# if001/lit-llama-ja

Hardware: AMD Instinct MI355X
Metric: decode tokens/sec LLaMA-7B gptq.int4 bs=1, 1xMI355X per replica (higher is better)
Workload: dtype bf16; 1 GPU; LLaMA-7B --quantize gptq.int4 greedy decode, batch 1, prompt 16, max_seq_length 144; batch_per_gpu=1, prompt_len=16, max_seq_length=144, parallelism=replicas x1 (no collective on the data path)

## Files before the change

### __graft_entry__.py

```python
from __future__ import annotations

import sys
from pathlib import Path

REPO = Path(__file__).resolve().parent
PKG_ROOT = REPO / "lit-llama-ja_amd"
for _p in (str(REPO), str(PKG_ROOT)):
    if _p not in sys.path:
        sys.path.insert(0, _p)


def build() -> None:
    from lit_llama._build import build as _build

    so = _build(force=True, verbose=True)
    import lit_llama
    from lit_llama import _hip

    L = _hip.lib()
    print(f"built {so} ({so.stat().st_size} bytes); {len(_hip.SIGNATURES) + len(_hip.LORA_SIGNATURES) + len(_hip.NLL_SIGNATURES) + 1} entry points resolved")


def smoke() -> None:
    import numpy as np
    import torch

    import generate as G
    from lit_llama import LLaMA, LLaMAConfig
    from lit_llama.utils import EmptyInitOnDevice
    from oracle import llama_np as O
    from oracle.weights import Cfg, make_params

    assert torch.cuda.is_available(), "smoke() needs the GPU"
    g = dict(np.load(REPO / "tests" / "golden" / "int4_gptq.npz"))
    cfg = Cfg(block_size=128, n_layer=2, n_head=4, n_embd=256, vocab_size=2048)
    params = make_params(cfg, int(g["seed"]))
    packed = {k[3:]: v for k, v in g.items() if k.startswith("sd/")}
    with EmptyInitOnDevice(device=torch.device("cuda:0"), dtype=torch.bfloat16, quantization_mode="gptq.int4"):
        model = LLaMA(LLaMAConfig(block_size=128, vocab_size=2048, n_layer=2, n_head=4, n_embd=256))
    sd = {k: torch.from_numpy(v) for k, v in params.items() if not (k.endswith(".weight") and "wte" not in k)}
    sd.update({k: torch.from_numpy(np.ascontiguousarray(v)) for k, v in packed.items()})
    model.load_state_dict(sd)
    prompt = torch.from_numpy(g["prompt"]).cuda()
    ids = G.generate(model, prompt, 8, top_k=1).cpu().numpy()
    ref = g["bf16_ids"][: len(ids)]
    assert (ids == ref).all(), f"greedy ids {ids} != reference {ref}"
    lin = {k[:-len(".quant_weight")]: O.LinearSpec("colblock", qw=v, scales=packed[k[:-12] + "scales"],
                                                    zeros=packed[k[:-12] + "zeros"], bits=4)
           for k, v in packed.items() if k.endswith(".quant_weight")}
    orc = O.OracleLLaMA(cfg, params, linears=lin)
    want = orc.forward(g["prompt"][None].astype(np.int64))[0, -1]
    model.reset_cache()
    got = model(prompt[None].long())[0, -1].float().cpu().numpy()
# ... 8 lines not shown
```

### include/lit_llama_amd.h

```cpp
#ifndef LIT_LLAMA_AMD_H
#define LIT_LLAMA_AMD_H

#include <stddef.h>

#ifdef __cplusplus
extern "C" {
#endif

#define LLJ_EINVAL 1000

int llj_w4_repack(const void* qweight_ref, void* packed, int N, int K, void* stream);
int llj_w4_unpack(const void* packed, void* qweight_ref, int N, int K, void* stream);

int llj_w4_scale_zero(const void* scales, const void* zeros, int dtype, void* sz, int N, void* stream);

int llj_w8_repack(const void* qweight_ref, void* packed, int N, int K, void* stream);
int llj_w8_unpack(const void* packed, void* qweight_ref, int N, int K, void* stream);
int llj_w8_scale_zero(const void* scales, const void* zeros, int dtype, void* sz, int N, void* stream);

int llj_i8_repack(const void* cb, void* packed, int N, int K, void* stream);
int llj_i8_unpack(const void* packed, void* cb, int N, int K, void* stream);

int llj_set_tpw_max(int tiles);

// ... 151 lines not shown
int llj_g_sample(const float* logits, int ldl, int M, int V, float temperature, int top_k, const float* u,
                 unsigned long long seed, int* out_idx, int* tokens_out, int tok_stride, const int* pos, void* stream);

size_t llj_i8_rowstats_bytes(int K);
int llj_attention_i8(const void* q, const void* kcache, const void* vcache, void* y, const int* pos, int B, int T,
                     int n_head, int head_size, int S, int nsplit, void* part_ws, void* y_stats, void* clr,
                     int clr_words, float threshold, void* stream);
int llj_i8_swiglu_stats(const void* x, const void* CB1, const void* SCB1, const void* CB2, const void* SCB2, void* h,
                        int M, int H, int K, const void* i8ws, const void* x_stats, void* h_stats, void* clr,
                        int clr_words, float threshold, void* stream);
#define LLJ_WF_I8_ROWSTATS 0x10000
int llj_i8_norm_rowstats(const void* x, const void* norm_w, float eps, void* xn, int M, int K, float threshold, void* ws,
                         void* st, void* stream);
int llj_i8_linear_resid(const void* A, int lda, const void* CB, const void* SCB, void* x, int ldx, int M, int N, int K,
                        const void* stats, void* stream);

int llj_attention_adapter(const void* q, const void* kcache, const void* vcache, void* y, const int* pos, int B, int T,
                          int n_head, int head_size, int S, const void* ak, const void* av, const float* gate, int aT,
                          void* stream);
int llj_adapter_prefix_add(const void* q, const void* ak, const void* av, const float* gate, void* y, int M, int n_head,
                           int head_size, int aT, int dt, void* stream);

int llj_stream_read(const void* p, size_t bytes, float* out, int grid, void* stream);


#ifdef __cplusplus
}
#endif

#include "lit_llama_amd_lora.h"

#include "lit_llama_amd_nll.h"

#endif
```

### lit-llama-ja_amd/csrc/gemv.hip

```cpp
#include "gemv_impl.h"

namespace llj {

int g_tpw_max = LLJ_TPW_MAX;
int g_stream_a = 1;

template <int EP>
static int dispatch(int wf, int am, const GemvParams& p, hipStream_t s) {
  if (p.lora.t) {
    if (EP != EP_QKV || p.ad_s) return LLJ_EINVAL;
    switch (wf) {
      case WF_W4: return gemv_launch_lora_w4(am, p, s);
      case WF_BF16: return gemv_launch_lora_bf16(am, p, s);
      case WF_W8: return gemv_launch_lora_w8(am, p, s);
      case WF_W4G: return gemv_launch_lora_w4g(am, p, s);
    }
    return LLJ_EINVAL;
  }
  if (p.ad_s) {
    switch (wf) {
      case WF_W4: return gemv_launch_aff_w4(am, EP, p, s);
      case WF_BF16: return gemv_launch_aff_bf16(am, EP, p, s);
      case WF_W8: return gemv_launch_aff_w8(am, EP, p, s);
      case WF_W4G: return gemv_launch_aff_w4g(am, EP, p, s);
// ... 40 lines not shown
  const int old = g_tpw_max;
  g_tpw_max = tiles < 1 ? 1 : tiles;
  return old;
}

int llj_set_stream_a(int mode) {
  const int old = g_stream_a;
  g_stream_a = mode < 0 ? 0 : mode > 2 ? 2 : mode;
  return old;
}

int llj_linear(int wfmt, const void* A, int lda, const void* W, const void* sz, const void* bias, void* C,
               int ldc, int M, int N, int K, const void* i8ws, int i8_row0, const float* rowsum, void* stream) {
  GemvParams p{};
  p.rowsum = rowsum;
  p.A = (const bf16_t*)A; p.lda = lda; p.M = M; p.N = N; p.K = K;
  p.W = W; p.sz = (const float2*)sz; p.bias = (const bf16_t*)bias; p.C = (bf16_t*)C; p.ldc = ldc;
  p.i8ws = i8ws; p.m0 = i8_row0;
  return run<EP_STORE>(wfmt, p, stream);
}

int llj_norm_linear(int wfmt, const void* x, const void* norm_w, float eps, const void* W, const void* sz,
                    void* out, int ldo, int M, int N, int K, const void* i8ws, int i8_row0, const float* rowsum,
                    const float* nstat, int npart, void* stream) {
  GemvParams p{};
  p.rowsum = rowsum;
  p.nstat = nstat; p.npart = npart;
  p.A = (const bf16_t*)x; p.lda = K; p.norm_w = (const bf16_t*)norm_w; p.eps = eps; p.M = M; p.N = N; p.K = K;
  p.W = W; p.sz = (const float2*)sz; p.C = (bf16_t*)out; p.ldc = ldo;
  p.i8ws = i8ws; p.m0 = i8_row0;
  return run<EP_STORE>(wfmt, p, stream);
}

int llj_linear_resid(int wfmt, const void* A, int lda, const void* W, const void* sz, void* x, int ldx, int M,
                     int N, int K, const void* i8ws, int i8_row0, float* nstat_out, void* stream) {
  GemvParams p{};
  p.nstat_out = nstat_out;
  p.A = (const bf16_t*)A; p.lda = lda; p.M = M; p.N = N; p.K = K;
  p.W = W; p.sz = (const float2*)sz; p.C = (bf16_t*)x; p.ldc = ldx;
  p.i8ws = i8ws; p.m0 = i8_row0;
  return run<EP_RESID>(wfmt, p, stream);
}

int llj_norm_swiglu(int wfmt, const void* x, const void* norm_w, float eps, const void* W1, const void* sz1,
                    const void* W2, const void* sz2, void* h, int M, int H, int K, const void* i8ws, int i8_row0,
                    const float* rowsum, const float* nstat, int npart, void* stream) {
  GemvParams p{};
  p.rowsum = rowsum;
  p.nstat = nstat; p.npart = npart;
  p.A = (const bf16_t*)x; p.lda = K; p.norm_w = (const bf16_t*)norm_w; p.eps = eps; p.M = M; p.N = H; p.K = K;
  p.W = W1; p.W2 = W2; p.sz = (const float2*)sz1; p.sz2 = (const float2*)sz2; p.C = (bf16_t*)h; p.ldc = H;
  p.i8ws = i8ws; p.m0 = i8_row0;
  return run<EP_SWIGLU>(wfmt, p, stream);
}

int llj_norm_qkv_rope(int wfmt, const void* x, const void* norm_w, float eps, const void* W, const void* sz,
                      void* q_out, void* kcache, void* vcache, const float* rope, const int* pos, int B, int T,
                      int C, int n_head, int S, int row0, int rows, const void* i8ws, const float* rowsum,
                      const float* nstat, int npart, void* stream) {
  GemvParams p{};
  p.rowsum = rowsum ? rowsum + row0 : nullptr;
  p.nstat = nstat ? nstat + row0 : nullptr; p.npart = npart;
  if (row0 < 0 || rows < 1 || row0 + rows > B * T || n_head < 1 || C % n_head || S < 1) return LLJ_EINVAL;
  p.A = (const bf16_t*)x + (size_t)row0 * C; p.lda = C; p.norm_w = (const bf16_t*)norm_w; p.eps = eps;
  p.M = rows; p.m0 = row0; p.N = 3 * C; p.K = C;
  p.W = W; p.sz = (const float2*)sz; p.q_out = (bf16_t*)q_out; p.kcache = (bf16_t*)kcache;
// ... 160 lines not shown
```

### lit-llama-ja_amd/csrc/gemv_impl.h

```cpp
#pragma once
#include <algorithm>

#include "common.h"
#include "i8ws.h"
#include "attention.h"
#include "lit_llama_amd.h"

namespace llj {

enum : int { WF_W4 = 0, WF_BF16 = 1, WF_I8 = 2, WF_W8 = 3, WF_W4G = 4 };
enum : int { AM_GLOBAL = 0, AM_LDS = 1, AM_NORM = 2, AM_STREAM = 3, AM_SNORM = 4, AM_I8Q = 5, AM_I8S = 6, AM_MERGE = 7 };
constexpr int kMergeMax = 4;
constexpr int kSRow = 136;
constexpr int kSSlot = 8 * kSRow;
__host__ __device__ constexpr bool am_stream(int am) { return am == AM_STREAM || am == AM_SNORM; }
constexpr int kQRow = 144;
constexpr int kQSlotBytes = 8 * kQRow + 128 * 32;
constexpr int kQSlotBytesS = 8 * kQRow;
enum : int { EP_STORE = 0, EP_RESID = 1, EP_QKV = 2, EP_SWIGLU = 3 };


struct GemvParams {
  const bf16_t* A;
  int lda;
// ... 2 lines not shown
  int M, N, K;
  const void* W;
  const void* W2;
  const float2* sz;
  const float2* sz2;
  const bf16_t* bias;
  bf16_t* C;
  int ldc;
  bf16_t* q_out;
  bf16_t* kcache;
  bf16_t* vcache;
  const float* rope;
  const int* pos;
  int n_head, head_size, S, T;
  int m0;
  const void* i8ws;
  const float* rowsum;
  const float* nstat;
  int npart;
  float* nstat_out;
  int gch;
  const uint32_t* i8st;
  uint32_t* i8st_out;
  uint32_t* clr;
  int clr_words;
  float thr;
  const float* apart;
  int asplit;
  const bf16_t* ad_s;
  const bf16_t* ad_b;
  const bf16_t* ad_s2;
  const bf16_t* ad_b2;
  LoraArgs lora;
};
constexpr int kNstRows = 16;

__device__ __forceinline__ float rms_rstd(float sumsq_over_k, float eps) {
  return round_bf(rsqrtf(round_bf(round_bf(sumsq_over_k) + eps)));
}

__device__ __forceinline__ uint4 norm8(uint4 x, uint4 g, float r) {
  uint32_t xw[4] = {x.x, x.y, x.z, x.w}, gw[4] = {g.x, g.y, g.z, g.w}, o[4];
#pragma unroll
  for (int i = 0; i < 4; ++i) o[i] = cvt_pk(unpk(gw[i]) * unpk(cvt_pk(unpk(xw[i]) * r)));
  return make_uint4(o[0], o[1], o[2], o[3]);
}
__device__ __forceinline__ f32x2 sumsq8(const u32x4 x, f32x2 acc) {
#pragma unroll
  for (int i = 0; i < 4; ++i) {
    const f32x2 v = unpk(x[i]);
    acc += unpk(cvt_pk(v * v));
  }
  return acc;
}

template <int NW, bool NORM>
__device__ void stage_a(const GemvParams& p, bf16_t* As, int a_stride, float* red) {
  const int tid = threadIdx.x;
  constexpr int NT = NW * 64;
  const int K = p.K, M = p.M;
  const int nvec = K >> 3;
  float ss[8];
#pragma unroll
  for (int m = 0; m < 8; ++m) ss[m] = 0.f;
  const bool from_stat = NORM && p.nstat;
#pragma unroll
// ... 1236 lines not shown
        const int b = p.T == 1 ? mg : mg / p.T;
        float out = v;
        if (region < 2) out = (dd & 1) ? (v * cs.x + partner * cs.y) : (v * cs.x - partner * cs.y);
        const uint32_t ob = (uint32_t)f2bf(out);
        const uint32_t pr = lane_xor1(ob);
        if (!(dd & 1)) {
          bf16_t* dst;
          size_t ei;
          if (region == 0) {
            dst = p.q_out;
            ei = (size_t)mg * Cd + nc;
          } else {
            int slot = ps;
            if (slot >= p.S) slot %= p.S;
            dst = region == 1 ? p.kcache : p.vcache;
            ei = (((size_t)b * p.n_head + h) * p.S + slot) * p.head_size + dd;
          }
          epi_store(dst + ei, ob | (pr << 16));
        }
      }
    } else if (EP == EP_RESID) {
      const float xn = round_bf(bf2f(xr) + round_bf(y));
      const uint32_t xb = (uint32_t)f2bf(xn);
      const uint32_t pr = lane_xor1(xb);
      if (act && !(row & 1)) epi_store(p.C + (size_t)m * p.ldc + n, xb | (pr << 16));
      if (p.nstat_out) {
        const float sq = row16_sum(act ? round_bf(xn * xn) : 0.f);
        if (row == 0 && act) epi_store(p.nstat_out + (size_t)nt * kNstRows + m, __builtin_bit_cast(uint32_t, sq));
      }
    } else {
      const uint32_t ob = (uint32_t)f2bf(out_value<EP>(y, y2));
      const uint32_t pr = lane_xor1(ob);
      if (act && !(row & 1)) epi_store(p.C + (size_t)m * p.ldc + n, ob | (pr << 16));
      if constexpr (EP == EP_SWIGLU && I8) {
        if (p.i8st_out) {
          const float a16 = fabsf(f16r(bflo(ob)));
          big = act && a16 >= p.thr;
          const float mx = row16_max(act && !big ? a16 : 0.f);
          if (row == 0 && act) atomicMax(p.i8st_out + kI8StSca + 8 * (nt % kI8StSlots) + m, __float_as_uint(mx));
        }
      }
    }
    return big;
  };

  if constexpr ((LLJ_ABL & 4) != 0) {
    if (wave == 0 && acc[0][0] == 1234.5f && row < M) p.C[nj[0]] = f2bf(acc[0][1] + acc2[0][2]);
  } else if constexpr (FLAT) {
#pragma unroll
    for (int q = 0; q < FQ; ++q) {
      const int j = f_j[q], m = f_m[q];
      const int src = ((m >> 2) << 4) | row, r = m & 3;
      float ya = 0.f, yb = 0.f, ys = 0.f;
      int yi = 0, yi2 = 0;
#pragma unroll
      for (int w = 0; w < NW; ++w) {
        const float* o = red + (size_t)(w * 64 + src) * NV;
        if constexpr (I8) {
          const int* oi = reinterpret_cast<const int*>(o);
          yi = w == 0 ? oi[r] : yi + oi[r];
          yi2 = w == 0 ? oi[4 + r] : yi2 + oi[4 + r];
        } else {
          ya = w == 0 ? o[8 * j + r] : ya + o[8 * j + r];
          if (DUAL) yb = w == 0 ? o[8 * j + 4 + r] : yb + o[8 * j + 4 + r];
          if (SACC) ys = w == 0 ? o[8 * TPW + r] : ys + o[8 * TPW + r];
        }
// ... 303 lines not shown
```

### lit-llama-ja_amd/csrc/ops.hip

```cpp
#include <cstdlib>

#include "common.h"
#include "attention.h"
#include "lit_llama_amd.h"

namespace llj {

__global__ __launch_bounds__(256) void embedding_kernel(const int* __restrict__ idx, const uint4* __restrict__ wte,
                                                        uint4* __restrict__ out, int C8, int* pos_inc) {
  const int m = blockIdx.x;
  const size_t r = (size_t)idx[m];
  for (int v = threadIdx.x; v < C8; v += blockDim.x) out[(size_t)m * C8 + v] = wte[r * C8 + v];
  if (pos_inc && m == 0 && threadIdx.x == 0) *pos_inc += 1;
}

__global__ __launch_bounds__(256) void embedding_any_kernel(const int* __restrict__ idx, const bf16_t* __restrict__ wte,
                                                            bf16_t* __restrict__ out, int C, int* pos_inc) {
  const int m = blockIdx.x;
  const size_t r = (size_t)idx[m];
  for (int v = threadIdx.x; v < C; v += blockDim.x) out[(size_t)m * C + v] = wte[r * C + v];
  if (pos_inc && m == 0 && threadIdx.x == 0) *pos_inc += 1;
}


// ... 62 lines not shown

template <int HS, int U, int NTH, int SPECU>
__global__ __launch_bounds__(NTH) void attention_kernel(const bf16_t* __restrict__ q, const bf16_t* __restrict__ kc,
                                                        const bf16_t* __restrict__ vc, bf16_t* __restrict__ y,
                                                        const int* __restrict__ pos, int T, int S, int nh,
                                                        float scale_log2, uint32_t* st, float thr, uint32_t* clr,
                                                        int clr_words, int spec_ok) {
  __shared__ float lds[attention_lds_floats<HS, NTH>()];
  attention_body<HS, U, NTH, false, SPECU>(q, kc, vc, y, pos, T, S, nh, scale_log2, blockIdx.x, blockIdx.y, lds, 1, 0,
                                           nullptr, st, thr, clr, clr_words, spec_ok != 0);
}

template <int HS, int U, int NTH>
__global__ __launch_bounds__(NTH) void attention_part_kernel(const bf16_t* __restrict__ q, const bf16_t* __restrict__ kc,
                                                             const bf16_t* __restrict__ vc, const int* __restrict__ pos,
                                                             int T, int S, int nh, float scale_log2, int nsplit,
                                                             float* __restrict__ part) {
  __shared__ float lds[attention_lds_floats<HS, NTH>()];
  attention_body<HS, U, NTH, true>(q, kc, vc, nullptr, pos, T, S, nh, scale_log2, blockIdx.x, blockIdx.y, lds, nsplit,
                                   blockIdx.z, part);
}

template <int HS, int U, int NTH, int SPECU>
__global__ __launch_bounds__(NTH) void attention_ilv_kernel(const bf16_t* __restrict__ q, const bf16_t* __restrict__ kc,
                                                            const bf16_t* __restrict__ vc, const int* __restrict__ pos,
                                                            int T, int S, int nh, float scale_log2, int nsplit,
                                                            float* __restrict__ part, int spec_ok) {
  __shared__ float lds[attention_lds_floats<HS, NTH>()];
  attention_body<HS, U, NTH, true, SPECU, true>(q, kc, vc, nullptr, pos, T, S, nh, scale_log2, blockIdx.x, blockIdx.y,
                                                lds, nsplit, blockIdx.z, part, nullptr, 0.f, nullptr, 0,
                                                spec_ok != 0);
}

__global__ __launch_bounds__(1024) void argmax_kernel(const bf16_t* __restrict__ logits, int ldl, int V,
                                                      int* __restrict__ out_idx, int* __restrict__ tokens_out,
                                                      int tok_stride, const int* __restrict__ pos) {
  __shared__ float sv[16];
  __shared__ int si[16];
  const int m = blockIdx.x, tid = threadIdx.x;
  const bf16_t* lr = logits + (size_t)m * ldl;
  float best = -INFINITY;
  int bi = 0x7fffffff;
  auto take = [&](float x, int v) {
    if (x > best || (x == best && v < bi)) { best = x; bi = v; }
  };
  if ((V & 7) == 0 && (ldl & 7) == 0 && (reinterpret_cast<uintptr_t>(lr) & 15) == 0) {
    const uint4* l4 = reinterpret_cast<const uint4*>(lr);
    const int nv = V >> 3;
    for (int v0 = tid; v0 < nv; v0 += 4 * 1024) {
      uint4 r[4];
#pragma unroll
      for (int u = 0; u < 4; ++u) {
        const int v = v0 + 1024 * u;
        r[u] = l4[v < nv ? v : v0];
      }
#pragma unroll
      for (int u = 0; u < 4; ++u) {
        const int v = v0 + 1024 * u;
        if (v < nv) {
          const uint32_t w[4] = {r[u].x, r[u].y, r[u].z, r[u].w};
#pragma unroll
          for (int i = 0; i < 4; ++i) {
            take(bflo(w[i]), 8 * v + 2 * i);
            take(bfhi(w[i]), 8 * v + 2 * i + 1);
          }
        }
      }
    }
  } else {
    for (int v = tid; v < V; v += 1024) take(bf2f(lr[v]), v);
  }
#pragma unroll
  for (int o = 32; o > 0; o >>= 1) {
    const float ov = __shfl_xor(best, o, 64);
    const int oi = __shfl_xor(bi, o, 64);
    if (ov > best || (ov == best && oi < bi)) { best = ov; bi = oi; }
  }
  if ((tid & 63) == 0) { sv[tid >> 6] = best; si[tid >> 6] = bi; }
  __syncthreads();
  if (tid == 0) {
    for (int w = 1; w < 16; ++w)
      if (sv[w] > best || (sv[w] == best && si[w] < bi)) { best = sv[w]; bi = si[w]; }
    if (bi == 0x7fffffff) bi = 0;
    out_idx[m] = bi;
    if (tokens_out) tokens_out[(size_t)m * tok_stride + pos[0] + 1] = bi;
  }
}


__device__ __forceinline__ uint32_t bf_key(uint32_t b) { return (b & 0x8000u) ? (~b & 0xFFFFu) : (b | 0x8000u); }
__device__ __forceinline__ float key_bf(uint32_t k) {
  const uint32_t b = (k & 0x8000u) ? (k & 0x7FFFu) : (~k & 0xFFFFu);
  return bf2f((bf16_t)b);
}
__device__ __forceinline__ uint64_t splitmix64(uint64_t z) {
  z += 0x9E3779B97F4A7C15ull;
  z = (z ^ (z >> 30)) * 0xBF58476D1CE4E5B9ull;
  z = (z ^ (z >> 27)) * 0x94D049BB133111EBull;
  return z ^ (z >> 31);
}

constexpr int kSampNT = 1024;
__device__ __forceinline__ uint32_t block_suffix_excl(uint32_t v, uint32_t* wsum) {
  const int lane = threadIdx.x & 63, wv = threadIdx.x >> 6;
  uint32_t x = v;
#pragma unroll
  for (int o = 1; o < 64; o <<= 1) {
    const uint32_t y = (uint32_t)__shfl_down((int)x, o, 64);
    if (lane + o < 64) x += y;
  }
  if (lane == 0) wsum[wv] = x;
  __syncthreads();
  uint32_t above = 0;
  for (int w = wv + 1; w < kSampNT / 64; ++w) above += wsum[w];
  __syncthreads();
  return x - v + above;
}

template <typename T>
struct SampTraits;
template <>
// ... 308 lines not shown
                     int clr_words, float threshold, void* stream) {
  LLJ_REQUIRE(y_stats && B * T <= 8 && clr_words >= 0 && (!clr_words || clr));
  return attention_split_run(q, kcache, vcache, y, pos, B, T, n_head, head_size, S, nsplit, part_ws,
                             (uint32_t*)y_stats, threshold, (uint32_t*)clr, clr_words, stream);
}

int llj_sample(const void* logits, int ldl, int M, int V, float temperature, int top_k, const float* u,
               unsigned long long seed, int* out_idx, int* tokens_out, int tok_stride, const int* pos, void* stream) {
  LLJ_REQUIRE(M > 0 && V > 0 && temperature > 0.f && (!tokens_out || pos) && (u || pos));
  hipLaunchKernelGGL(sample_kernel<bf16_t>, dim3(M), dim3(kSampNT), 0, (hipStream_t)stream, (const bf16_t*)logits, ldl,
                     V, 1.f / temperature, temperature, top_k, u, (uint64_t)seed, out_idx, tokens_out, tok_stride, pos);
  LLJ_CHECK_LAUNCH();
  return 0;
}

int llj_g_sample(const float* logits, int ldl, int M, int V, float temperature, int top_k, const float* u,
                 unsigned long long seed, int* out_idx, int* tokens_out, int tok_stride, const int* pos, void* stream) {
  LLJ_REQUIRE(logits && out_idx && M > 0 && V > 0 && ldl >= V && temperature > 0.f && (!tokens_out || pos) && (u || pos));
  hipLaunchKernelGGL(sample_kernel<float>, dim3(M), dim3(kSampNT), 0, (hipStream_t)stream, logits, ldl, V,
                     1.f / temperature, temperature, top_k, u, (uint64_t)seed, out_idx, tokens_out, tok_stride, pos);
  LLJ_CHECK_LAUNCH();
  return 0;
}

int llj_argmax(const void* logits, int ldl, int M, int V, int* out_idx, int* tokens_out, int tok_stride,
               const int* pos, void* stream) {
  LLJ_REQUIRE(M > 0 && V > 0 && (!tokens_out || pos));
  hipLaunchKernelGGL(argmax_kernel, dim3(M), dim3(1024), 0, (hipStream_t)stream, (const bf16_t*)logits, ldl, V,
                     out_idx, tokens_out, tok_stride, pos);
  LLJ_CHECK_LAUNCH();
  return 0;
}

}
```

### lit-llama-ja_amd/lit_llama/_hip.py

```python
from __future__ import annotations

import ctypes
import os
from pathlib import Path

import torch

LIB_PATH = Path(os.environ["LLJ_LIB"]) if os.environ.get("LLJ_LIB") else Path(__file__).resolve().parent / "_lljamd.so"

_P = ctypes.c_void_p
_I = ctypes.c_int
_F = ctypes.c_float


SIGNATURES = {
    "llj_w4_repack": [_P, _P, _I, _I, _P],
    "llj_w4_unpack": [_P, _P, _I, _I, _P],
    "llj_w4_scale_zero": [_P, _P, _I, _P, _I, _P],
    "llj_w8_repack": [_P, _P, _I, _I, _P],
    "llj_w8_unpack": [_P, _P, _I, _I, _P],
    "llj_i8_repack": [_P, _P, _I, _I, _P],
    "llj_i8_unpack": [_P, _P, _I, _I, _P],
    "llj_w8_scale_zero": [_P, _P, _I, _P, _I, _P],
    "llj_linear": [_I, _P, _I, _P, _P, _P, _P, _I, _I, _I, _I, _P, _I, _P, _P],
# ... 48 lines not shown
    "llj_g_argmax": [_P, _I, _I, _I, _P, _P, _I, _P, _P],
    "llj_g_sample": [_P, _I, _I, _I, _F, _I, _P, ctypes.c_ulonglong, _P, _P, _I, _P, _P],
    "llj_g_i8_linear": [_P, _I, _I, _I, _P, _P, _F, _P, _I, _P, _I, _P, _I, _I, _P],
    "llj_attention_adapter": [_P, _P, _P, _P, _P, _I, _I, _I, _I, _I, _P, _P, _P, _I, _P],
    "llj_adapter_prefix_add": [_P, _P, _P, _P, _P, _I, _I, _I, _I, _I, _P],
    "llj_linear_v2": [_I, _P, _I, _P, _P, _P, _P, _I, _I, _I, _I, _P, _I, _P, _P, _P, _P],
    "llj_norm_qkv_rope_v2": [_I, _P, _P, _F, _P, _P, _P, _P, _P, _P, _P, _I, _I, _I, _I, _I, _I, _I, _P, _P, _P, _I,
                             _P, _P, _P],
    "llj_linear_resid_v2": [_I, _P, _I, _P, _P, _P, _I, _I, _I, _I, _P, _I, _P, _P, _P, _P],
    "llj_linear_resid_attn_v2": [_I, _P, _I, _I, _P, _P, _P, _I, _I, _I, _P, _P, _P, _P],
    "llj_norm_swiglu_v2": [_I, _P, _P, _F, _P, _P, _P, _P, _P, _I, _I, _I, _P, _I, _P, _P, _I, _P, _P, _P, _P, _P],
    "llj_norm_linear_v2": [_I, _P, _P, _F, _P, _P, _P, _I, _I, _I, _I, _P, _I, _P, _P, _I, _P, _P, _P],
    "llj_gemm_linear_v2": [_I, _P, _I, _P, _P, _P, _I, _I, _I, _I, _P, _P, _P],
    "llj_gemm_resid_v2": [_I, _P, _I, _P, _P, _P, _I, _I, _I, _I, _P, _P, _P],
    "llj_gemm_silu_mul_v2": [_I, _P, _I, _P, _P, _P, _I, _I, _I, _I, _P, _P, _P],
    "llj_gemm_qkv_rope_v2": [_I, _P, _P, _P, _P, _P, _P, _P, _P, _I, _I, _I, _I, _I, _P, _P, _P],
    "llj_g_linear_v2": [_I, _P, _I, _I, _I, _P, _P, _P, _I, _I, _I, _P, _I, _P, _I, _I, _P, _P, _P],
}

LORA_SIGNATURES = {
    "llj_lora_merge": [_P, _P, _P, _I, _I, _I, _I, _F, _I, _I, _P],
    "llj_norm_qkv_rope_lora": [_I, _P, _P, _F, _P, _P, _P, _P, _P, _P, _P, _I, _I, _I, _I, _I, _I, _I, _P, _P, _P,
                               _I, _P, _P, _I, _P, _I, _I, _F],
    "llj_gemm_qkv_rope_lora": [_I, _P, _P, _P, _P, _P, _P, _P, _P, _I, _I, _I, _I, _I, _P, _P, _I, _P, _I, _I, _F],
    "llj_g_linear_lora": [_I, _P, _I, _I, _I, _P, _P, _P, _I, _I, _I, _P, _I, _P, _I, _I, _P, _P, _I, _P, _I, _I,
                          _F],
}

NLL_SIGNATURES = {
    "llj_nll": [_P, _I, _I, _I, _P, _P, _P, _P],
    "llj_g_nll": [_P, _I, _I, _I, _P, _P, _P, _P],
}

_lib = None


class HipError(RuntimeError):
    pass


WF_I8_ROWSTATS = 0x10000
WF_ZINT = 0x20000
(OPT_ATT_SPEC_FULL, OPT_FLASH_QB, OPT_FLASH_PAIR, OPT_GEMM_GLDS, OPT_GLDS_COST128, OPT_GEMV_LDS_A_KB,
 OPT_ATT_SPEC_BATCH, OPT_GEMM_W4Z) = range(8)


def lib() -> ctypes.CDLL:
    global _lib
    if _lib is None:
        if not LIB_PATH.exists():
            raise HipError(
                f"{LIB_PATH} is missing: build it with `python -c 'import __graft_entry__ as g; g.build()'` "
                "(hipcc --offload-arch=gfx950). There is no fallback path.")
        L = ctypes.CDLL(str(LIB_PATH))
        for name, argt in {**SIGNATURES, **LORA_SIGNATURES, **NLL_SIGNATURES}.items():
            f = getattr(L, name)
            f.argtypes = argt
            f.restype = ctypes.c_int
        L.llj_i8_ws_bytes.argtypes = [_I, _I]
        L.llj_i8_ws_bytes.restype = ctypes.c_size_t
        L.llj_attention_ws_bytes.argtypes = [_I, _I, _I, _I]
        L.llj_attention_ws_bytes.restype = ctypes.c_size_t
        L.llj_g_i8_ws_bytes.argtypes = [_I, _I]
        L.llj_g_i8_ws_bytes.restype = ctypes.c_size_t
        L.llj_i8_rowstats_bytes.argtypes = [_I]
        L.llj_i8_rowstats_bytes.restype = ctypes.c_size_t
        L.llj_gemm_resid_ws_bytes.argtypes = [_I, _I, _I, _I]
        L.llj_gemm_resid_ws_bytes.restype = ctypes.c_size_t
        L.llj_gemm_swiglu_ws_bytes.argtypes = [_I, _I, _I, _I]
        L.llj_gemm_swiglu_ws_bytes.restype = ctypes.c_size_t
        _lib = L
    return _lib


def call(name: str, *args) -> None:
    rc = getattr(lib(), name)(*args)
    if rc != 0:
        what = "unsupported shape/argument (EINVAL)" if rc == 1000 else f"hipError {rc}"
        raise HipError(f"{name} failed: {what}")


def stream() -> int:
    return torch.cuda.current_stream().cuda_stream


def require_device(t: torch.Tensor, what: str = "tensor") -> None:
    if t.device.type != "cuda" or torch.version.hip is None:
        raise HipError(
# ... 7 lines not shown
```

### lit-llama-ja_amd/lit_llama/engine.py

```python
from __future__ import annotations

import torch

from . import _hip
from .model import LLaMA, _Work


class DecodeSession:
    def __init__(self, model: LLaMA, batch: int, max_seq_length: int, total_len: int, use_graph: bool = True,
                 temperature: float = 1.0, top_k: int | None = 1, seed: int = 0,
                 uniforms: torch.Tensor | None = None):
        cfg = model.config
        assert max_seq_length <= cfg.block_size
        self.model, self.B, self.S, self.total = model, batch, max_seq_length, total_len
        dev = model.transformer.wte.weight.device
        _hip.require_device(model.transformer.wte.weight, "model")
        self.dev = dev
        if batch < 1:
            raise ValueError(f"decode batch {batch} < 1")
        self.cur = torch.zeros(batch, dtype=torch.int32, device=dev)
        self.pos = torch.zeros(1, dtype=torch.int32, device=dev)
        self.tokens = torch.zeros(batch, total_len, dtype=torch.int32, device=dev)
        self.logits = torch.empty(batch, cfg.padded_vocab_size, dtype=model.act_dtype(), device=dev)
        self.use_graph = use_graph
        self.graph = None
        self.t_prompt = 0
        self.steps_done = 0
        self.specs = None
        self.work = None
        self.temperature = float(temperature)
        self.top_k = 0 if top_k is None else int(top_k)
        self.seed = int(seed) & ((1 << 64) - 1)
        if uniforms is not None:
            assert uniforms.dtype == torch.float32 and uniforms.shape == (total_len, batch) and uniforms.is_contiguous()
            _hip.require_device(uniforms, "uniforms")
        self.uniforms = uniforms

    def _choose(self, st):
        cfg = self.model.config
        if self.logits.dtype == torch.float32 and self.top_k != 1:
            _hip.call("llj_g_sample", self.logits.data_ptr(), self.logits.stride(0), self.B, cfg.padded_vocab_size,
                      self.temperature, self.top_k, _hip.ptr(self.uniforms), self.seed, self.cur.data_ptr(),
                      self.tokens.data_ptr(), self.total, self.pos.data_ptr(), st)
        elif self.logits.dtype == torch.float32:
            _hip.call("llj_g_argmax", self.logits.data_ptr(), self.logits.stride(0), self.B, cfg.padded_vocab_size,
                      self.cur.data_ptr(), self.tokens.data_ptr(), self.total, self.pos.data_ptr(), st)
        elif self.top_k == 1:
            _hip.call("llj_argmax", self.logits.data_ptr(), self.logits.stride(0), self.B, cfg.padded_vocab_size,
                      self.cur.data_ptr(), self.tokens.data_ptr(), self.total, self.pos.data_ptr(), st)
        else:
            _hip.call("llj_sample", self.logits.data_ptr(), self.logits.stride(0), self.B, cfg.padded_vocab_size,
                      self.temperature, self.top_k, _hip.ptr(self.uniforms), self.seed, self.cur.data_ptr(),
                      self.tokens.data_ptr(), self.total, self.pos.data_ptr(), st)

    @torch.no_grad()
    def prefill(self, prompts: torch.Tensor) -> None:
        m = self.model
        B, T = prompts.shape
        assert B == self.B and T + 1 <= self.total
        m.reset_cache()
        m.kv_caches = m._alloc_kv(B, self.S, self.dev)
        if m.rope_cache is None:
            m.rope_cache = m.build_rope_cache(prompts)
        pos = torch.arange(T, device=self.dev, dtype=torch.int32)
        m._run(prompts.to(self.dev), pos, self.S, m.kv_caches, last_only_out=self.logits)
        st = _hip.stream()
        self.tokens[:, :T] = prompts.to(torch.int32)
        self.pos.fill_(T - 1)
        self._choose(st)
        self.t_prompt = T
        self.steps_done = 1
        self.specs = m._layer_specs()
        if m._generic():
            self.work = _Work(m.config, B, self.dev, False, self.S, generic=True, dtype=m.act_dtype(),
                              lora_cols=self.specs.get("lora_cols", 0))
        else:
            need_i8 = any(s[0] == 2 for layer in self.specs["layers"] for s in layer) or self.specs["head"][0] == 2
            self.work = _Work(m.config, B, self.dev, need_i8, self.S, lora_cols=self.specs.get("lora_cols", 0))
            m._enable_i8_handoff(self.work, self.specs)
        self.graph = None

    def _reset_handoff(self):
        w = self.work
        if w is not None and getattr(w, "y_st", None) is not None:
            w.y_st.zero_()
            w.h_st.zero_()

    def _step(self):
        try:
            self._step_launches()
        except BaseException:
            self._reset_handoff()
            raise

    def _step_launches(self):
        m, w, B = self.model, self.work, self.B
        cfg = m.config
        st = _hip.stream()
        if w.generic:
            _hip.call("llj_g_embedding", self.cur.data_ptr(), m.transformer.wte.weight.data_ptr(), w.x.data_ptr(), B,
                      cfg.n_embd, self.pos.data_ptr(), w.dt, st)
        else:
            _hip.call("llj_embedding", self.cur.data_ptr(), m.transformer.wte.weight.data_ptr(), w.x.data_ptr(), B,
                      cfg.n_embd, self.pos.data_ptr(), st)
        m._blocks(w, self.specs, m.kv_caches, self.pos, B, 1, self.S, st)
        m._head(w.x, B, self.specs, self.logits, st, w)
        self._choose(st)

    def capture(self):
        if self.graph is not None or not self.use_graph:
            return
        g = torch.cuda.CUDAGraph()
        with torch.cuda.graph(g):
            self._step()
        self.graph = g

    @torch.no_grad()
    def decode(self, n: int) -> None:
        assert self.t_prompt + self.steps_done + n <= self.total, "beyond the output buffer"
        assert self.t_prompt + self.steps_done + n - 1 <= self.model.config.block_size, "beyond block_size"
        if self.use_graph:
            self.capture()
            for _ in range(n):
                self.graph.replay()
        else:
            for _ in range(n):
                self._step()
        self.steps_done += n

    def output(self) -> torch.Tensor:
        return self.tokens[:, :self.t_prompt + self.steps_done]
```

### lit-llama-ja_amd/lit_llama/model.py

```python
from __future__ import annotations

import math
import os
import types
from dataclasses import dataclass
from typing import List, Optional, Tuple

import torch
import torch.nn as nn
from typing_extensions import Self

from . import _hip
from .utils import find_multiple

MaskCache = torch.Tensor
RoPECache = torch.Tensor
KVCache = Tuple[torch.Tensor, torch.Tensor]


@dataclass
class LLaMAConfig:
    block_size: int = 2048
    vocab_size: int = 32000
    padded_vocab_size: Optional[int] = None
# ... 17 lines not shown
            return f"n_embd {self.n_embd} is not a multiple of 128 (the GEMV K chunk)"
        if hs not in (64, 128):
            return f"head_size {hs} is not 64 or 128 (fused RoPE / attention kernels)"
        return None

    def debug(self):
        for k in ("block_size", "vocab_size", "padded_vocab_size", "n_layer", "n_head", "n_embd"):
            print(f"{k}: ", getattr(self, k))


llama_configs = {
    "19M": dict(n_layer=6, n_head=8, n_embd=512, vocab_size=35000),
    "49M": dict(n_layer=10, n_head=10, n_embd=640, vocab_size=35000),
    "125M": dict(n_layer=12, n_head=10, n_embd=780, vocab_size=35000),
    "7B": dict(n_layer=32, n_head=32, n_embd=4096),
    "13B": dict(n_layer=40, n_head=40, n_embd=5120),
    "30B": dict(n_layer=60, n_head=52, n_embd=6656),
    "65B": dict(n_layer=80, n_head=64, n_embd=8192),
}

QKV_ROWS = 8
LIN_ROWS = 16
I8_ROWS = 8
if os.environ.get("LLJ_I8_ROWS"):
    I8_ROWS = max(1, min(8, int(os.environ["LLJ_I8_ROWS"])))
ATTN_SPLIT_MIN_S = 512
ATTN_SPLIT_KEYS = 256


FLASH_MIN_T = 32


ATT_MERGE = 0


def attn_splits(S: int) -> int:
    if S < ATTN_SPLIT_MIN_S:
        return 1
    return min(64, (S + ATTN_SPLIT_KEYS - 1) // ATTN_SPLIT_KEYS)
PRE_NORM_ROWS = True
PRE_NORM_MIN_M = 2
HAND_NORM = True
HAND_NORM_MAX_M = 8
HAND_NORM_MIN_M = 2


GEMM_MIN_ROWS = 32
_GEMM_FMTS = (0, 1, 2, 3, 4)


def _gemm_fmt(wfmt: int) -> bool:
    return (wfmt & 0xFF) in _GEMM_FMTS


GEMM_ZINT = True
GEMM_SWIGLU = True


def _gz(wfmt: int, lin: nn.Module) -> int:
    if GEMM_ZINT and wfmt == 0 and hasattr(lin, "zeros_integral") and lin.zeros_integral():
        return wfmt | _hip.WF_ZINT
    return wfmt

I8_GATHER = True
I8_GATHER_BUDGET = 256 << 20
I8_GATHER_MAX = 16256
# ... 623 lines not shown
                rs = w.rs if f1 in _ROWSUM_FMTS else None
                _hip.call("llj_rmsnorm_rows", w.x.data_ptr(), blk.rms_2.scale.data_ptr(), blk.rms_2.eps,
                          w.xn.data_ptr(), P(rs), M, C, st)
                src, nw, step = w.xn, None, QKV_ROWS
            else:
                src, nw, step = w.x, blk.rms_2.scale.data_ptr(), QKV_ROWS
            nst = w.nst if (w.hand and f1 != 2) else None
            if w.i8s and not w.flash:
                ns = I8_NORM_ROWSTATS
                _hip.call("llj_i8_swiglu_stats", src.data_ptr(), w1.data_ptr(), P(s1), w2.data_ptr(), P(s2),
                          w.h.data_ptr(), M, H, C, None if ns else w.i8ws.data_ptr(), w.n_st.data_ptr() if ns else None,
                          w.h_st.data_ptr(), w.y_st.data_ptr(), w.y_st.numel(), Linear8bitLtThreshold, st)
                _hip.call("llj_i8_linear_resid", w.h.data_ptr(), H, wd.data_ptr(), P(sd), w.x.data_ptr(), C, M, C, H,
                          w.h_st.data_ptr(), st)
                continue
            for r0 in range(0, M, step):
                r = min(step, M - r0)
                _lcall("llj_norm_swiglu", a12, f1, src[r0].data_ptr(), nw, blk.rms_2.eps, w1.data_ptr(), P(s1),
                       w2.data_ptr(), P(s2), w.h[r0].data_ptr(), r, H, C, P(w.i8ws), r0,
                       None if rs is None else rs[r0].data_ptr(), None if nst is None else nst[r0].data_ptr(),
                       w.npart, st)
            self._resid(fd, w.h, wd, sd, w.x, M, C, H, w, st, w.nst if w.hand else None, ad)

    def _resid(self, f, A, W, sz, x, M, N, K, w, st, nst=None, af=None):
        if f == 2:
            self._i8_prep(A, M, K, w, st)
        step = I8_ROWS if f == 2 else LIN_ROWS
        for r0 in range(0, M, step):
            r = min(step, M - r0)
            _lcall("llj_linear_resid", af, f, A[r0].data_ptr(), A.stride(0), W.data_ptr(), _hip.ptr(sz),
                   x[r0].data_ptr(), x.stride(0), r, N, K, _hip.ptr(w.i8ws), r0,
                   None if nst is None else nst[r0].data_ptr(), st)

    def _head(self, x, M, specs, out, st, w):
        cfg = self.config
        C, V = cfg.n_embd, cfg.padded_vocab_size
        ln = self.transformer.ln_f
        if w.generic:
            xn = w.xn if M <= w.xn.shape[0] else torch.empty_like(x)
            _hip.call("llj_g_rmsnorm", x.data_ptr(), x.stride(0), ln.scale.data_ptr(), ln.eps, xn.data_ptr(), C, M, C,
                      w.dt, st)
            self._glinear(specs["head"], xn, M, C, V, out, None, st, specs.get("head_affine"))
            return
        f, W, sz = specs["head"]
        ah = specs.get("head_affine")
        rs = nst = None
        if f == 2 and w.i8s and I8_NORM_ROWSTATS and x is w.x:
            xn = w.xn
            _hip.call("llj_i8_norm_rowstats", x.data_ptr(), ln.scale.data_ptr(), ln.eps, xn.data_ptr(), M, C,
                      Linear8bitLtThreshold, w.i8ws.data_ptr(), w.n_st.data_ptr(), st)
            _hip.call("llj_norm_linear", f | _hip.WF_I8_ROWSTATS, xn.data_ptr(), None, ln.eps, W.data_ptr(),
                      _hip.ptr(sz), out.data_ptr(), out.stride(0), M, V, C, w.n_st.data_ptr(), 0, None, None, 0, st)
            return
        if f == 2:
            xn = torch.empty_like(x)
            self._i8_norm_prep(x, ln, xn, M, C, w, st)
            if M >= GEMM_MIN_ROWS and C % 128 == 0 and V % 128 == 0:
                ao, (wg,), kp = self._i8_gathered(xn, M, C, [(W, sz, V)], w, st)
                _hip.call("llj_gemm_i8_linear", xn.data_ptr(), C, W.data_ptr(), _hip.ptr(sz), _hip.ptr(w.i8ws),
                          _hip.ptr(ao), _hip.ptr(wg), kp, out.data_ptr(), out.stride(0), M, V, C, st)
                return
            src, nw = xn, None
        elif M >= GEMM_MIN_ROWS and _gemm_fmt(f) and C % 128 == 0 and V % 128 == 0:
            xn = torch.empty_like(x)
            _hip.call("llj_rmsnorm_rows", x.data_ptr(), ln.scale.data_ptr(), ln.eps, xn.data_ptr(), None, M, C, st)
            _lcall("llj_gemm_linear", ah, _gz(f, self.lm_head), xn.data_ptr(), C, W.data_ptr(), _hip.ptr(sz),
                   out.data_ptr(), out.stride(0), M, V, C, st)
            return
        elif x is w.x and w.hand and f != 2 and len(self.transformer.h) > 0:
            nst = w.nst
            src, nw = x, ln.scale.data_ptr()
        elif M >= 2 and w.pre:
            xn = torch.empty_like(x)
            rs = torch.empty(M, dtype=torch.float32, device=x.device) if f in _ROWSUM_FMTS else None
            _hip.call("llj_rmsnorm_rows", x.data_ptr(), ln.scale.data_ptr(), ln.eps, xn.data_ptr(), _hip.ptr(rs), M,
                      C, st)
            src, nw = xn, None
        else:
            src, nw = x, ln.scale.data_ptr()
        for r0 in range(0, M, QKV_ROWS):
            r = min(QKV_ROWS, M - r0)
            _lcall("llj_norm_linear", ah, f, src[r0].data_ptr(), nw, ln.eps, W.data_ptr(), _hip.ptr(sz),
                   out[r0].data_ptr(), out.stride(0), r, V, C, _hip.ptr(w.i8ws), r0,
                   None if rs is None else rs[r0].data_ptr(), None if nst is None else nst[r0].data_ptr(),
                   w.npart, st)


Linear8bitLtThreshold = 6.0


class Block(nn.Module):

    def __init__(self, config: LLaMAConfig) -> None:
        super().__init__()
        self.rms_1 = RMSNorm(config.n_embd)
        self.attn = CausalSelfAttention(config)
        self.rms_2 = RMSNorm(config.n_embd)
        self.mlp = MLP(config)
        self.config = config

    def forward(self, x, rope, mask, max_seq_length, input_pos=None, kv_cache=None):
        if input_pos is not None or kv_cache is not None:
            raise NotImplementedError("Block.forward with a KV cache runs inside LLaMA.forward(idx, max_seq_length, "
                                      "input_pos) on this path")
        B, T, C = x.shape
        _hip.require_device(x, "x")
        cfg = self.config
        model = _BlockHost(self, cfg)
        return model.run(x, rope), None


class _BlockHost:

    def __init__(self, blk, cfg):
        self.blk, self.cfg = blk, cfg

    def run(self, x, rope):
        blk, cfg = self.blk, self.cfg
# ... 172 lines not shown
```

Before: 896.9 tokens/s.

## Fuse per-tile argmax into LM head and merge greedy choose with embedding

The LM-head GEMV epilogue now writes a per-16-column tile max and its index. A new choose_embed kernel reduces those tile maxima instead of rescanning the full vocab logits, falls back to a full scan when NaNs are present, and writes the chosen token's embedding row straight into the next step's activation buffer. This drops the separate embedding launch and most of the argmax memory traffic per decode step. In exchange the GEMV epilogue does extra cross-lane reductions, and a ticket atomic advances pos when M>1.

```diff
diff --git a/__graft_entry__.py b/__graft_entry__.py
--- a/__graft_entry__.py
+++ b/__graft_entry__.py
@@ -18,7 +18,7 @@
     from lit_llama import _hip
 
     L = _hip.lib()
-    print(f"built {so} ({so.stat().st_size} bytes); {len(_hip.SIGNATURES) + len(_hip.LORA_SIGNATURES) + len(_hip.NLL_SIGNATURES) + 1} entry points resolved")
+    print(f"built {so} ({so.stat().st_size} bytes); {len(_hip.SIGNATURES) + len(_hip.LORA_SIGNATURES) + len(_hip.NLL_SIGNATURES) + len(_hip.DECODE_SIGNATURES) + 1} entry points resolved")
 
 
 def smoke() -> None:
diff --git a/include/lit_llama_amd.h b/include/lit_llama_amd.h
--- a/include/lit_llama_amd.h
+++ b/include/lit_llama_amd.h
@@ -207,4 +207,6 @@
 
 #include "lit_llama_amd_nll.h"
 
+#include "lit_llama_amd_decode.h"
+
 #endif
diff --git a/include/lit_llama_amd_decode.h b/include/lit_llama_amd_decode.h
--- /dev/null
+++ b/include/lit_llama_amd_decode.h
@@ -0,0 +1,19 @@
+#ifndef LIT_LLAMA_AMD_DECODE_H
+#define LIT_LLAMA_AMD_DECODE_H
+
+#ifdef __cplusplus
+extern "C" {
+#endif
+
+int llj_norm_linear_tmax(int wfmt, const void* x, const void* norm_w, float eps, const void* W, const void* sz,
+                         void* out, int ldo, int M, int N, int K, const void* i8ws, int i8_row0, const float* rowsum,
+                         const float* nstat, int npart, void* tmax, void* stream);
+
+int llj_choose_embed(const void* logits, int ldl, int M, int V, const void* tmax, int* out_idx, int* tokens_out,
+                     int tok_stride, int* pos, const void* wte, void* x, int C, int* ticket, void* stream);
+
+#ifdef __cplusplus
+}
+#endif
+
+#endif
diff --git a/lit-llama-ja_amd/csrc/gemv.hip b/lit-llama-ja_amd/csrc/gemv.hip
--- a/lit-llama-ja_amd/csrc/gemv.hip
+++ b/lit-llama-ja_amd/csrc/gemv.hip
@@ -96,6 +96,20 @@
   return run<EP_STORE>(wfmt, p, stream);
 }
 
+int llj_norm_linear_tmax(int wfmt, const void* x, const void* norm_w, float eps, const void* W, const void* sz,
+                         void* out, int ldo, int M, int N, int K, const void* i8ws, int i8_row0, const float* rowsum,
+                         const float* nstat, int npart, void* tmax, void* stream) {
+  if (M > 8 || (N & 15) || (reinterpret_cast<uintptr_t>(tmax) & 7)) return LLJ_EINVAL;
+  GemvParams p{};
+  p.rowsum = rowsum;
+  p.nstat = nstat; p.npart = npart;
+  p.A = (const bf16_t*)x; p.lda = K; p.norm_w = (const bf16_t*)norm_w; p.eps = eps; p.M = M; p.N = N; p.K = K;
+  p.W = W; p.sz = (const float2*)sz; p.C = (bf16_t*)out; p.ldc = ldo;
+  p.i8ws = i8ws; p.m0 = i8_row0;
+  p.tmax = (float2*)tmax;
+  return run<EP_STORE>(wfmt, p, stream);
+}
+
 int llj_linear_resid(int wfmt, const void* A, int lda, const void* W, const void* sz, void* x, int ldx, int M,
                      int N, int K, const void* i8ws, int i8_row0, float* nstat_out, void* stream) {
   GemvParams p{};
diff --git a/lit-llama-ja_amd/csrc/gemv_impl.h b/lit-llama-ja_amd/csrc/gemv_impl.h
--- a/lit-llama-ja_amd/csrc/gemv_impl.h
+++ b/lit-llama-ja_amd/csrc/gemv_impl.h
@@ -58,6 +58,7 @@
   const bf16_t* ad_s2;
   const bf16_t* ad_b2;
   LoraArgs lora;
+  float2* tmax;
 };
 constexpr int kNstRows = 16;
 
@@ -1360,6 +1361,18 @@
       const uint32_t ob = (uint32_t)f2bf(out_value<EP>(y, y2));
       const uint32_t pr = lane_xor1(ob);
       if (act && !(row & 1)) epi_store(p.C + (size_t)m * p.ldc + n, ob | (pr << 16));
+      if constexpr (EP == EP_STORE) {
+        if (p.tmax) {
+          const float v = bflo(ob);
+          const bool isn = v != v;
+          const bool anyn = row16_max(isn ? 1.f : 0.f) > 0.f;
+          const float mx = row16_max(isn ? -INFINITY : v);
+          const bool hit = anyn ? isn : v == mx;
+          const int first = 15 - (int)row16_max(hit ? (float)(15 - row) : -1.f);
+          if (row == 0 && act)
+            p.tmax[(size_t)m * ntiles + nt] = make_float2(anyn ? __int_as_float(0x7fc00000) : mx, __int_as_float(n0 + first));
+        }
+      }
       if constexpr (EP == EP_SWIGLU && I8) {
         if (p.i8st_out) {
           const float a16 = fabsf(f16r(bflo(ob)));
diff --git a/lit-llama-ja_amd/csrc/ops.hip b/lit-llama-ja_amd/csrc/ops.hip
--- a/lit-llama-ja_amd/csrc/ops.hip
+++ b/lit-llama-ja_amd/csrc/ops.hip
@@ -118,61 +118,142 @@
                                                 spec_ok != 0);
 }
 
+struct ArgBest {
+  float best = -INFINITY;
+  int bi = 0x7fffffff;
+  __device__ __forceinline__ void take(float x, int v) {
+    if (x > best || (x == best && v < bi)) { best = x; bi = v; }
+  }
+};
+
+__device__ __forceinline__ void argmax_scan(const bf16_t* __restrict__ lr, int ldl, int V, int tid, ArgBest& a) {
+  if ((V & 7) == 0 && (ldl & 7) == 0 && (reinterpret_cast<uintptr_t>(lr) & 15) == 0) {
+    const uint4* l4 = reinterpret_cast<const uint4*>(lr);
+    const int nv = V >> 3;
+    for (int v0 = tid; v0 < nv; v0 += 4 * 1024) {
+      uint4 r[4];
+#pragma unroll
+      for (int u = 0; u < 4; ++u) {
+        const int v = v0 + 1024 * u;
+        r[u] = l4[v < nv ? v : v0];
+      }
+#pragma unroll
+      for (int u = 0; u < 4; ++u) {
+        const int v = v0 + 1024 * u;
+        if (v < nv) {
+          const uint32_t w[4] = {r[u].x, r[u].y, r[u].z, r[u].w};
+#pragma unroll
+          for (int i = 0; i < 4; ++i) {
+            a.take(bflo(w[i]), 8 * v + 2 * i);
+            a.take(bfhi(w[i]), 8 * v + 2 * i + 1);
+          }
+        }
+      }
+    }
+  } else {
+    for (int v = tid; v < V; v += 1024) a.take(bf2f(lr[v]), v);
+  }
+}
+
+__device__ __forceinline__ void argmax_reduce(ArgBest& a, int tid, float* sv, int* si) {
+#pragma unroll
+  for (int o = 32; o > 0; o >>= 1) {
+    const float ov = __shfl_xor(a.best, o, 64);
+    const int oi = __shfl_xor(a.bi, o, 64);
+    a.take(ov, oi);
+  }
+  if ((tid & 63) == 0) { sv[tid >> 6] = a.best; si[tid >> 6] = a.bi; }
+  __syncthreads();
+  if (tid == 0) {
+    for (int w = 1; w < 16; ++w) a.take(sv[w], si[w]);
+    if (a.bi == 0x7fffffff) a.bi = 0;
+  }
+}
+
 __global__ __launch_bounds__(1024) void argmax_kernel(const bf16_t* __restrict__ logits, int ldl, int V,
                                                       int* __restrict__ out_idx, int* __restrict__ tokens_out,
                                                       int tok_stride, const int* __restrict__ pos) {
   __shared__ float sv[16];
   __shared__ int si[16];
   const int m = blockIdx.x, tid = threadIdx.x;
-  const bf16_t* lr = logits + (size_t)m * ldl;
-  float best = -INFINITY;
-  int bi = 0x7fffffff;
-  auto take = [&](float x, int v) {
-    if (x > best || (x == best && v < bi)) { best = x; bi = v; }
-  };
-  if ((V & 7) == 0 && (ldl & 7) == 0 && (reinterpret_cast<uintptr_t>(lr) & 15) == 0) {
-    const uint4* l4 = reinterpret_cast<const uint4*>(lr);
-    const int nv = V >> 3;
-    for (int v0 = tid; v0 < nv; v0 += 4 * 1024) {
-      uint4 r[4];
-#pragma unroll
-      for (int u = 0; u < 4; ++u) {
-        const int v = v0 + 1024 * u;
-        r[u] = l4[v < nv ? v : v0];
+  ArgBest a;
+  argmax_scan(logits + (size_t)m * ldl, ldl, V, tid, a);
+  argmax_reduce(a, tid, sv, si);
+  if (tid == 0) {
+    out_idx[m] = a.bi;
+    if (tokens_out) tokens_out[(size_t)m * tok_stride + pos[0] + 1] = a.bi;
+  }
+}
+
+__global__ __launch_bounds__(1024) void choose_embed_kernel(const bf16_t* __restrict__ logits, int ldl, int V,
+                                                            const float2* __restrict__ tmax, int* __restrict__ out_idx,
+                                                            int* __restrict__ tokens_out, int tok_stride,
+                                                            int* __restrict__ pos, const uint4* __restrict__ wte,
+                                                            uint4* __restrict__ x, int C8, int* __restrict__ ticket) {
+  __shared__ float sv[16];
+  __shared__ int si[16];
+  __shared__ int sn[16];
+  __shared__ int s_tok;
+  const int m = blockIdx.x, tid = threadIdx.x;
+  const int nt = V >> 4;
+  int p = 0;
+  if (tid == 0) p = pos[0];
+  bool scan = !tmax;
+  ArgBest a;
+  if (tmax) {
+    const float2* tr = tmax + (size_t)m * nt;
+    int nan = 0;
+    for (int i0 = tid; i0 < nt; i0 += 2 * 1024) {
+      const int i1 = i0 + 1024;
+      const float2 r0 = tr[i0], r1 = tr[i1 < nt ? i1 : i0];
+      nan |= r0.x != r0.x;
+      a.take(r0.x, __float_as_int(r0.y));
+      if (i1 < nt) {
+        nan |= r1.x != r1.x;
+        a.take(r1.x, __float_as_int(r1.y));
       }
-#pragma unroll
-      for (int u = 0; u < 4; ++u) {
-        const int v = v0 + 1024 * u;
-        if (v < nv) {
-          const uint32_t w[4] = {r[u].x, r[u].y, r[u].z, r[u].w};
-#pragma unroll
-          for (int i = 0; i < 4; ++i) {
-            take(bflo(w[i]), 8 * v + 2 * i);
-            take(bfhi(w[i]), 8 * v + 2 * i + 1);
-          }
-        }
+    }
+    nan = __any(nan);
+#pragma unroll
+    for (int o = 32; o > 0; o >>= 1) {
+      const float ov = __shfl_xor(a.best, o, 64);
+      const int oi = __shfl_xor(a.bi, o, 64);
+      a.take(ov, oi);
+    }
+    if ((tid & 63) == 0) { sv[tid >> 6] = a.best; si[tid >> 6] = a.bi; sn[tid >> 6] = nan; }
+    __syncthreads();
+    if (tid == 0) {
+      for (int w = 1; w < 16; ++w) {
+        a.take(sv[w], si[w]);
+        nan |= sn[w];
       }
-    }
-  } else {
-    for (int v = tid; v < V; v += 1024) take(bf2f(lr[v]), v);
-  }
-#pragma unroll
-  for (int o = 32; o > 0; o >>= 1) {
-    const float ov = __shfl_xor(best, o, 64);
-    const int oi = __shfl_xor(bi, o, 64);
-    if (ov > best || (ov == best && oi < bi)) { best = ov; bi = oi; }
-  }
-  if ((tid & 63) == 0) { sv[tid >> 6] = best; si[tid >> 6] = bi; }
-  __syncthreads();
+      s_tok = nan ? -1 : a.bi;
+    }
+    __syncthreads();
+    scan = s_tok < 0;
+  }
+  if (scan) {
+    a = ArgBest();
+    argmax_scan(logits + (size_t)m * ldl, ldl, V, tid, a);
+    argmax_reduce(a, tid, sv, si);
+    if (tid == 0) s_tok = a.bi;
+    __syncthreads();
+  }
+  const int tok = s_tok;
   if (tid == 0) {
-    for (int w = 1; w < 16; ++w)
-      if (sv[w] > best || (sv[w] == best && si[w] < bi)) { best = sv[w]; bi = si[w]; }
-    if (bi == 0x7fffffff) bi = 0;
-    out_idx[m] = bi;
-    if (tokens_out) tokens_out[(size_t)m * tok_stride + pos[0] + 1] = bi;
-  }
-}
-
+    out_idx[m] = tok;
+    if (tokens_out) tokens_out[(size_t)m * tok_stride + p + 1] = tok;
+    bool last = true;
+    if (gridDim.x > 1) {
+      __threadfence();
+      last = atomicAdd(ticket, 1) == (int)gridDim.x - 1;
+      if (last) *ticket = 0;
+    }
+    if (last) pos[0] = p + 1;
+  }
+  const size_t r = (size_t)tok;
+  for (int v = tid; v < C8; v += 1024) x[(size_t)m * C8 + v] = wte[r * C8 + v];
+}
 
 __device__ __forceinline__ uint32_t bf_key(uint32_t b) { return (b & 0x8000u) ? (~b & 0xFFFFu) : (b | 0x8000u); }
 __device__ __forceinline__ float key_bf(uint32_t k) {
@@ -547,4 +628,15 @@
   return 0;
 }
 
-}
+int llj_choose_embed(const void* logits, int ldl, int M, int V, const void* tmax, int* out_idx, int* tokens_out,
+                     int tok_stride, int* pos, const void* wte, void* x, int C, int* ticket, void* stream) {
+  LLJ_REQUIRE(logits && out_idx && pos && wte && x && M > 0 && V > 0 && ldl >= V && C > 0 && C % 8 == 0);
+  LLJ_REQUIRE((M == 1 || ticket) && (!tmax || V % 16 == 0));
+  hipLaunchKernelGGL(choose_embed_kernel, dim3(M), dim3(1024), 0, (hipStream_t)stream, (const bf16_t*)logits, ldl, V,
+                     (const float2*)tmax, out_idx, tokens_out, tok_stride, pos, (const uint4*)wte, (uint4*)x, C / 8,
+                     ticket);
+  LLJ_CHECK_LAUNCH();
+  return 0;
+}
+
+}
diff --git a/lit-llama-ja_amd/lit_llama/_hip.py b/lit-llama-ja_amd/lit_llama/_hip.py
--- a/lit-llama-ja_amd/lit_llama/_hip.py
+++ b/lit-llama-ja_amd/lit_llama/_hip.py
@@ -104,6 +104,11 @@
     "llj_g_nll": [_P, _I, _I, _I, _P, _P, _P, _P],
 }
 
+DECODE_SIGNATURES = {
+    "llj_norm_linear_tmax": [_I, _P, _P, _F, _P, _P, _P, _I, _I, _I, _I, _P, _I, _P, _P, _I, _P, _P],
+    "llj_choose_embed": [_P, _I, _I, _I, _P, _P, _P, _I, _P, _P, _P, _I, _P, _P],
+}
+
 _lib = None
 
 
@@ -125,7 +130,7 @@
                 f"{LIB_PATH} is missing: build it with `python -c 'import __graft_entry__ as g; g.build()'` "
                 "(hipcc --offload-arch=gfx950). There is no fallback path.")
         L = ctypes.CDLL(str(LIB_PATH))
-        for name, argt in {**SIGNATURES, **LORA_SIGNATURES, **NLL_SIGNATURES}.items():
+        for name, argt in {**SIGNATURES, **LORA_SIGNATURES, **NLL_SIGNATURES, **DECODE_SIGNATURES}.items():
             f = getattr(L, name)
             f.argtypes = argt
             f.restype = ctypes.c_int
diff --git a/lit-llama-ja_amd/lit_llama/engine.py b/lit-llama-ja_amd/lit_llama/engine.py
--- a/lit-llama-ja_amd/lit_llama/engine.py
+++ b/lit-llama-ja_amd/lit_llama/engine.py
@@ -3,6 +3,7 @@
 import torch
 
 from . import _hip
+from . import model as MD
 from .model import LLaMA, _Work
 
 
@@ -24,6 +25,9 @@
         self.logits = torch.empty(batch, cfg.padded_vocab_size, dtype=model.act_dtype(), device=dev)
         self.use_graph = use_graph
         self.graph = None
+        self.fused_tail = False
+        self.tmax = None
+        self.ticket = torch.zeros(1, dtype=torch.int32, device=dev)
         self.t_prompt = 0
         self.steps_done = 0
         self.specs = None
@@ -53,6 +57,13 @@
                       self.temperature, self.top_k, _hip.ptr(self.uniforms), self.seed, self.cur.data_ptr(),
                       self.tokens.data_ptr(), self.total, self.pos.data_ptr(), st)
 
+    def _choose_embed(self, st, tmax):
+        cfg = self.model.config
+        _hip.call("llj_choose_embed", self.logits.data_ptr(), self.logits.stride(0), self.B, cfg.padded_vocab_size,
+                  _hip.ptr(tmax), self.cur.data_ptr(), self.tokens.data_ptr(), self.total, self.pos.data_ptr(),
+                  self.model.transformer.wte.weight.data_ptr(), self.work.x.data_ptr(), cfg.n_embd,
+                  self.ticket.data_ptr(), st)
+
     @torch.no_grad()
     def prefill(self, prompts: torch.Tensor) -> None:
         m = self.model
@@ -67,7 +78,6 @@
         st = _hip.stream()
         self.tokens[:, :T] = prompts.to(torch.int32)
         self.pos.fill_(T - 1)
-        self._choose(st)
         self.t_prompt = T
         self.steps_done = 1
         self.specs = m._layer_specs()
@@ -78,6 +88,15 @@
             need_i8 = any(s[0] == 2 for layer in self.specs["layers"] for s in layer) or self.specs["head"][0] == 2
             self.work = _Work(m.config, B, self.dev, need_i8, self.S, lora_cols=self.specs.get("lora_cols", 0))
             m._enable_i8_handoff(self.work, self.specs)
+        w = self.work
+        self.fused_tail = bool(MD.CHOOSE_EMBED and self.top_k == 1 and not w.generic and w.i8ws is None
+                               and self.logits.dtype == torch.bfloat16)
+        if self.fused_tail:
+            V = m.config.padded_vocab_size
+            self.tmax = torch.empty(B, V // 16, 2, dtype=torch.float32, device=self.dev) if V % 16 == 0 else None
+            self._choose_embed(st, None)
+        else:
+            self._choose(st)
         self.graph = None
 
     def _reset_handoff(self):
@@ -97,15 +116,21 @@
         m, w, B = self.model, self.work, self.B
         cfg = m.config
         st = _hip.stream()
-        if w.generic:
+        if self.fused_tail:
+            pass
+        elif w.generic:
             _hip.call("llj_g_embedding", self.cur.data_ptr(), m.transformer.wte.weight.data_ptr(), w.x.data_ptr(), B,
                       cfg.n_embd, self.pos.data_ptr(), w.dt, st)
         else:
             _hip.call("llj_embedding", self.cur.data_ptr(), m.transformer.wte.weight.data_ptr(), w.x.data_ptr(), B,
                       cfg.n_embd, self.pos.data_ptr(), st)
         m._blocks(w, self.specs, m.kv_caches, self.pos, B, 1, self.S, st)
-        m._head(w.x, B, self.specs, self.logits, st, w)
-        self._choose(st)
+        if self.fused_tail:
+            wrote = m._head(w.x, B, self.specs, self.logits, st, w, tmax=self.tmax)
+            self._choose_embed(st, self.tmax if wrote else None)
+        else:
+            m._head(w.x, B, self.specs, self.logits, st, w)
+            self._choose(st)
 
     def capture(self):
         if self.graph is not None or not self.use_graph:
diff --git a/lit-llama-ja_amd/lit_llama/model.py b/lit-llama-ja_amd/lit_llama/model.py
--- a/lit-llama-ja_amd/lit_llama/model.py
+++ b/lit-llama-ja_amd/lit_llama/model.py
@@ -73,6 +73,9 @@
 
 
 ATT_MERGE = 0
+
+
+CHOOSE_EMBED = 1
 
 
 def attn_splits(S: int) -> int:
@@ -762,7 +765,7 @@
                    x[r0].data_ptr(), x.stride(0), r, N, K, _hip.ptr(w.i8ws), r0,
                    None if nst is None else nst[r0].data_ptr(), st)
 
-    def _head(self, x, M, specs, out, st, w):
+    def _head(self, x, M, specs, out, st, w, tmax=None) -> bool:
         cfg = self.config
         C, V = cfg.n_embd, cfg.padded_vocab_size
         ln = self.transformer.ln_f
@@ -771,7 +774,7 @@
             _hip.call("llj_g_rmsnorm", x.data_ptr(), x.stride(0), ln.scale.data_ptr(), ln.eps, xn.data_ptr(), C, M, C,
                       w.dt, st)
             self._glinear(specs["head"], xn, M, C, V, out, None, st, specs.get("head_affine"))
-            return
+            return False
         f, W, sz = specs["head"]
         ah = specs.get("head_affine")
         rs = nst = None
@@ -781,7 +784,7 @@
                       Linear8bitLtThreshold, w.i8ws.data_ptr(), w.n_st.data_ptr(), st)
             _hip.call("llj_norm_linear", f | _hip.WF_I8_ROWSTATS, xn.data_ptr(), None, ln.eps, W.data_ptr(),
                       _hip.ptr(sz), out.data_ptr(), out.stride(0), M, V, C, w.n_st.data_ptr(), 0, None, None, 0, st)
-            return
+            return False
         if f == 2:
             xn = torch.empty_like(x)
             self._i8_norm_prep(x, ln, xn, M, C, w, st)
@@ -789,14 +792,14 @@
                 ao, (wg,), kp = self._i8_gathered(xn, M, C, [(W, sz, V)], w, st)
                 _hip.call("llj_gemm_i8_linear", xn.data_ptr(), C, W.data_ptr(), _hip.ptr(sz), _hip.ptr(w.i8ws),
                           _hip.ptr(ao), _hip.ptr(wg), kp, out.data_ptr(), out.stride(0), M, V, C, st)
-                return
+                return False
             src, nw = xn, None
         elif M >= GEMM_MIN_ROWS and _gemm_fmt(f) and C % 128 == 0 and V % 128 == 0:
             xn = torch.empty_like(x)
             _hip.call("llj_rmsnorm_rows", x.data_ptr(), ln.scale.data_ptr(), ln.eps, xn.data_ptr(), None, M, C, st)
             _lcall("llj_gemm_linear", ah, _gz(f, self.lm_head), xn.data_ptr(), C, W.data_ptr(), _hip.ptr(sz),
                    out.data_ptr(), out.stride(0), M, V, C, st)
-            return
+            return False
         elif x is w.x and w.hand and f != 2 and len(self.transformer.h) > 0:
             nst = w.nst
             src, nw = x, ln.scale.data_ptr()
@@ -808,12 +811,17 @@
             src, nw = xn, None
         else:
             src, nw = x, ln.scale.data_ptr()
+        tm = tmax is not None and ah is None and f != 2 and V % 16 == 0
         for r0 in range(0, M, QKV_ROWS):
             r = min(QKV_ROWS, M - r0)
-            _lcall("llj_norm_linear", ah, f, src[r0].data_ptr(), nw, ln.eps, W.data_ptr(), _hip.ptr(sz),
-                   out[r0].data_ptr(), out.stride(0), r, V, C, _hip.ptr(w.i8ws), r0,
-                   None if rs is None else rs[r0].data_ptr(), None if nst is None else nst[r0].data_ptr(),
-                   w.npart, st)
+            args = (f, src[r0].data_ptr(), nw, ln.eps, W.data_ptr(), _hip.ptr(sz), out[r0].data_ptr(), out.stride(0),
+                    r, V, C, _hip.ptr(w.i8ws), r0, None if rs is None else rs[r0].data_ptr(),
+                    None if nst is None else nst[r0].data_ptr(), w.npart)
+            if tm:
+                _hip.call("llj_norm_linear_tmax", *args, tmax[r0].data_ptr(), st)
+            else:
+                _lcall("llj_norm_linear", ah, *args, st)
+        return tm
 
 
 Linear8bitLtThreshold = 6.0
```

Result: no change. 901.0 tokens/s (median of 6 runs) (+0.5%).
